# zhiyongggggg/dct-cryptonets

Measured on AMD Instinct MI355X. Metric: encrypted images/sec, ResNet-20 DCT-24x16^2 CIFAR-10, higher is better.
Workload: dtype u64 torus + f64 FFT (one-level tiers keep 32-bit accumulators)

## Files before the change

### dct-cryptonets_amd/csrc/dctfhe.hip

```cpp
#include <hip/hip_runtime.h>
#include <sys/random.h>

#include <algorithm>
#include <array>
#include <atomic>
#include <cmath>
#include <cstdarg>
#include <cstddef>
#include <cstdio>
#include <cstring>
#include <map>
#include <memory>
#include <string>
#include <vector>

#include "../../include/dctfhe.h"
#include "kernels.h"

using namespace dctfhe;

static thread_local std::string g_err;
static int fail(const char* fmt, ...) {
  char buf[1024];
  va_list ap;
// ... 350 lines not shown
  ~dctfhe_session() {
    if (ctx) hipSetDevice(ctx->device);
    wipe_audit_key();
  }
};

#define PBS_CASES(X)                                                                                 \
  X(8, 2, 2, 8) X(9, 1, 2, 16) X(9, 1, 3, 8) X(10, 1, 1, 8) X(10, 1, 2, 8) X(10, 2, 1, 8) X(10, 2, 2, 8)  \
  X(11, 1, 1, 8) X(11, 1, 2, 8) X(11, 1, 3, 8) X(12, 1, 1, 8) X(12, 1, 2, 8) X(12, 1, 3, 8)           \
  X(13, 1, 1, 8) X(13, 1, 2, 8) X(13, 1, 3, 8) X(11, 1, 4, 8)

#define PBS_MB_CASES(X) X(11) X(12) X(13)

template <int LOGN, int K_, int L_, int P>
constexpr int groups_for() {
  using G = pbs_geom<LOGN, K_, L_, P>;
  constexpr int by_lds = (160 * 1024 - G::TW_BYTES) / G::GROUP_BYTES;
  int g = G::T >= 256 ? 1 : 256 / G::T;
  while (g > 1 && g > by_lds) g >>= 1;
  while (g > 1 && 2 * (G::TW_BYTES + g * G::GROUP_BYTES) > 160 * 1024) g >>= 1;
  return g;
}

static int tier_ppt(const dctfhe_tier& t) {
#define X(LN, K_, L_, P_) if (t.logN == LN && t.k == K_ && t.l == L_) return P_;
  PBS_CASES(X)
#undef X
  return 0;
}

#define SET_LDS_ATTR(kernel, bytes)                                                                  \
  do {                                                                                               \
    static uint64_t done_mask = 0;                                                                   \
    int dev_ = 0;                                                                                    \
    HIPCHK(hipGetDevice(&dev_));                                                                     \
    if (dev_ < 0 || dev_ >= 64 || !((done_mask >> dev_) & 1)) {                                      \
      HIPCHK(hipFuncSetAttribute((const void*)(kernel), hipFuncAttributeMaxDynamicSharedMemorySize, (int)(bytes))); \
      if (dev_ >= 0 && dev_ < 64) done_mask |= 1ull << dev_;                                         \
    }                                                                                                \
  } while (0)

template <int LN, int K, int L, int P, int GR, int MB = 0>
static int launch_pbs_as(const pbs_launch& a, hipStream_t st) {
  const size_t lds = pbs_lds_bytes<LN, K, L, P, MB>(GR);
  SET_LDS_ATTR((pbs_kernel<LN, K, L, P, GR, MB>), lds);
  const unsigned grid = (unsigned)((a.count + GR - 1) / GR);
  hipLaunchKernelGGL((pbs_kernel<LN, K, L, P, GR, MB>), dim3(grid), dim3(pbs_geom<LN, K, L, P, MB>::T * GR), lds, st, a);
  HIPCHK(hipGetLastError());
  return 0;
}

static int launch_pbs(const dctfhe_tier& t, const pbs_launch& a, hipStream_t st) {
  if (a.count == 0) return 0;
  if (a.pf_parts != 0 && a.pf_parts < 8) return fail("bootstrap launch: pf_parts must be 0 or >= 8 (got %d)", a.pf_parts);
  if (!a.bsk || !a.tw || !a.cts_small || !a.out || !a.dummy || (t.unroll == 2 && !a.wtab)) return fail("bootstrap launch: null operand");
  if (a.w < 0 || a.w > t.logN - 1) return fail("bootstrap launch: table of 2^%d entries does not fit N = 2^%d", a.w, t.logN);
#define X(LN, K_, L_, P_) \
  if (t.logN == LN && t.k == K_ && t.l == L_ && t.unroll == 1) return launch_pbs_as<LN, K_, L_, P_, groups_for<LN, K_, L_, P_>()>(a, st);
  PBS_CASES(X)
#undef X
#define X(LN) \
  if (t.logN == LN && t.k == 1 && t.l == 1 && t.unroll == 2) return launch_pbs_as<LN, 1, 1, 8, (LN == 12 ? 2 : groups_for<LN, 1, 1, 8>()), 1>(a, st);
  PBS_MB_CASES(X)
#undef X
  if (t.logN == 11 && t.k == 1 && t.l == 3 && t.unroll == 2) return launch_pbs_as<11, 1, 3, 8, 4, 1>(a, st);
  if (t.logN == 10 && t.k == 2 && t.l == 1 && t.unroll == 2) return launch_pbs_as<10, 2, 1, 8, 4, 1>(a, st);
  return fail("no bootstrap kernel instantiated for logN=%d k=%d l=%d unroll=%d", t.logN, t.k, t.l, t.unroll);
}

static int make_twiddles(const dctfhe_tier& t, std::vector<cplx>& tw) {
#define X(LN, K_, L_, P_)                                        \
  if (t.logN == LN && t.k == K_ && t.l == L_) {                  \
    tw.resize(fft_geom<LN - 1, P_>::TW_ELEMS);                   \
    fill_twiddles<LN - 1, P_>(tw.data());                        \
    return 0;                                                    \
  }
  PBS_CASES(X)
#undef X
  return fail("no bootstrap kernel instantiated for logN=%d k=%d l=%d", t.logN, t.k, t.l);
}

static int launch_bsk_fourier(const dctfhe_tier& t, const uint64_t* polys, size_t npoly, const cplx* tw, cplx* out, hipStream_t st) {
#define X(LN, K_, L_, P_)                                                                            \
  if (t.logN == LN && t.k == K_ && t.l == L_) {                                                      \
    using F = fft_geom<LN - 1, P_>;                                                                  \
    constexpr int GR = groups_for<LN, K_, L_, P_>();                                                 \
    const size_t lds = (size_t)F::TW_ELEMS * 16 + (size_t)GR * F::EXCH_ELEMS * 16;                   \
    SET_LDS_ATTR((k_bsk_fourier<LN, P_, GR>), lds);                                                  \
    const unsigned grid = (unsigned)((npoly + GR - 1) / GR);                                         \
    hipLaunchKernelGGL((k_bsk_fourier<LN, P_, GR>), dim3(grid), dim3(F::T * GR), lds, st, polys, npoly, tw, out); \
    HIPCHK(hipGetLastError());                                                                       \
    return 0;                                                                                        \
  }
  PBS_CASES(X)
#undef X
  return fail("no bootstrap kernel instantiated for logN=%d k=%d l=%d", t.logN, t.k, t.l);
}

extern "C" int dctfhe_ctx_create(int device_id, dctfhe_ctx** out) {
  int ndev = 0;
  if (hipGetDeviceCount(&ndev) != hipSuccess || ndev <= 0)
    return fail("dctfhe: no HIP device visible -- this engine has no CPU path");
  if (device_id < 0 || device_id >= ndev) return fail("dctfhe: device %d out of range (%d visible)", device_id, ndev);
  HIPCHK(hipSetDevice(device_id));
  std::unique_ptr<dctfhe_ctx> c(new dctfhe_ctx);
// ... 275 lines not shown
    if (t.ksk_share < 0) n += tier_ksk_words(p, t) * 8;
    n += tier_bsk_elems(t) * sizeof(cplx);
  }
  return n;
}
extern "C" int dctfhe_eval_keys_export(dctfhe_eval_keys* E, void* buf, size_t capacity, size_t* size) {
  if (!E || !size) return fail("dctfhe_eval_keys_export: null argument");
  const size_t need = eval_blob_size(E->p);
  *size = need;
  if (!buf) return 0;
  if (capacity < need) return fail("dctfhe_eval_keys_export: buffer of %zu bytes, %zu needed", capacity, need);
  HIPCHK(hipSetDevice(E->ctx->device));
  HIPCHK(hipStreamSynchronize(E->ctx->stream));
  EvalBlobHeader h{};
  h.magic = 0x4b564544u ; h.version = EVAL_BLOB_VERSION; h.total_bytes = need; h.params = E->p;
  char* q = (char*)buf;
  memcpy(q, &h, sizeof h); q += sizeof h;
  for (int ti = 0; ti < E->p.n_tiers; ti++) {
    const dctfhe_tier& t = E->p.tiers[ti];
    if (t.ksk_share < 0) {
      HIPCHK(hipMemcpy(q, E->ksk[ti].ksk.p, tier_ksk_words(E->p, t) * 8, hipMemcpyDeviceToHost));
      q += tier_ksk_words(E->p, t) * 8;
    }
    HIPCHK(hipMemcpy(q, E->tiers[ti].bsk.p, tier_bsk_elems(t) * sizeof(cplx), hipMemcpyDeviceToHost));
    q += tier_bsk_elems(t) * sizeof(cplx);
  }
  return 0;
}
static constexpr uint32_t EVAL_CBLOB_MAGIC = 0x43564544u , EVAL_CBLOB_VERSION = 1;
static size_t eval_cblob_size(const dctfhe_params& p) {
  size_t n = sizeof(EvalBlobHeader) + 32;
  for (int ti = 0; ti < p.n_tiers; ti++) {
    const dctfhe_tier& t = p.tiers[ti];
    if (t.ksk_share < 0) n += (size_t)p.D * t.lk * 8;
    n += tier_bsk_body_words(t) * 8;
  }
  return n;
}
static void key_to_bytes(const rng_key& k, uint8_t* b) {
  for (int i = 0; i < 8; i++) for (int x = 0; x < 4; x++) b[4 * i + x] = (uint8_t)(k.k[i] >> (8 * x));
}
static uint64_t ksk_grid_mask(const dctfhe_tier& t) {
  const int drop = 64 - 8 * ks_limbs(t);
  return drop ? ~0ULL << drop : ~0ULL;
}
static int launch_expand(const rng_key& key, uint64_t stream, uint64_t row0, uint64_t stride, int dim_eff, uint64_t and_mask, const uint64_t* d_bodies,
                         int nb, size_t count, size_t L, uint64_t* d_out, hipStream_t st) {
// ... 132 lines not shown
  CHK(expand_bsk_chunk(pub, tier, t, 0, (int)tier_bsk_blocks(t), (const uint64_t*)q, d_b.as<uint64_t>(), d_std.as<uint64_t>(), ctx->stream));
  HIPCHK(d_std.download(out, body_bytes * (t.k + 1), ctx->stream));
  return 0;
}

extern "C" int dctfhe_eval_keys_import(dctfhe_ctx* ctx, const void* buf, size_t size, dctfhe_eval_keys** out) {
  if (!ctx || !buf || !out) return fail("dctfhe_eval_keys_import: null argument");
  if (size < sizeof(EvalBlobHeader)) return fail("evaluation-key blob too short");
  EvalBlobHeader h;
  memcpy(&h, buf, sizeof h);
  if (h.magic == EVAL_CBLOB_MAGIC) return import_compressed(ctx, buf, size, out);
  if (h.magic != 0x4b564544u || h.version != EVAL_BLOB_VERSION) return fail("bad evaluation-key blob magic/version");
  CHK(check_params(&h.params));
  if (h.total_bytes != size || eval_blob_size(h.params) != size) return fail("evaluation-key blob is %zu bytes, its parameters need %zu", size, eval_blob_size(h.params));
  std::unique_ptr<dctfhe_eval_keys> E;
  CHK(eval_alloc(ctx, &h.params, E));
  const char* q = (const char*)buf + sizeof h;
  for (int ti = 0; ti < h.params.n_tiers; ti++) {
    const dctfhe_tier& t = h.params.tiers[ti];
    if (t.ksk_share < 0) {
      HIPCHK(hipMemcpy(E->ksk[ti].ksk.p, q, tier_ksk_words(h.params, t) * 8, hipMemcpyHostToDevice));
      q += tier_ksk_words(h.params, t) * 8;
    }
    HIPCHK(hipMemcpy(E->tiers[ti].bsk.p, q, tier_bsk_elems(t) * sizeof(cplx), hipMemcpyHostToDevice));
    q += tier_bsk_elems(t) * sizeof(cplx);
  }
  CHK(eval_finish(E.get()));
  *out = E.release();
  return 0;
}

extern "C" int dctfhe_client_key_export_secret(dctfhe_client_key* C, uint8_t* big_key, uint8_t* small_key) {
  HIPCHK(hipSetDevice(C->ctx->device));
  HIPCHK(hipMemcpy(big_key, C->S(), C->p.D, hipMemcpyDeviceToHost));
  HIPCHK(hipMemcpy(small_key, C->s(), C->p.n_max, hipMemcpyDeviceToHost));
  return 0;
}
extern "C" int dctfhe_eval_keys_export_ksk(dctfhe_eval_keys* K, int tier, uint64_t* out) {
  if (tier < 0 || tier >= K->p.n_tiers) return fail("tier out of range");
  const dctfhe_tier& t = K->p.tiers[tier];
  HIPCHK(hipSetDevice(K->ctx->device));
  HIPCHK(hipMemcpy(out, K->tiers[tier].ks->ksk.p, (size_t)K->p.D * t.lk * (t.n + 1) * 8, hipMemcpyDeviceToHost));
  return 0;
}
extern "C" int dctfhe_client_key_export_bsk(dctfhe_client_key* C, int tier, uint64_t* out) {
  if (tier < 0 || tier >= C->p.n_tiers) return fail("tier out of range");
  const dctfhe_tier& t = C->p.tiers[tier];
// ... 2365 lines not shown
```

### dct-cryptonets_amd/csrc/fft_core.h

```cpp
#pragma once
#include <stdint.h>
#include <type_traits>

#if defined(__HIPCC__)
#define HD __host__ __device__ __forceinline__
#else
#define HD inline __attribute__((always_inline))
#endif

namespace dctfhe {

struct cplx { double re, im; };

struct no_tick { template <int K> HD void at() {} };
#if defined(__HIP_DEVICE_COMPILE__) && defined(DCTFHE_PHASE_TIMERS)
struct phase_clock {
  unsigned long long last, acc[12];
  __device__ __forceinline__ void start() { for (int k = 0; k < 12; k++) acc[k] = 0; last = __builtin_amdgcn_s_memtime(); }
  template <int K> __device__ __forceinline__ void at() { const unsigned long long now = __builtin_amdgcn_s_memtime(); acc[K] += now - last; last = now; }
};
#endif

HD cplx cmk(double re, double im) { cplx c; c.re = re; c.im = im; return c; }
HD cplx cadd(cplx a, cplx b) { return cmk(a.re + b.re, a.im + b.im); }
// ... 66 lines not shown
      y[0] = cadd(a, b); y[1] = csub(a, b);
    } else {
      cplx e[R / 2], o[R / 2];
      small_dft<R / 2, 2 * S, SIGN>::run(x, e);
      small_dft<R / 2, 2 * S, SIGN>::run(x + S, o);
      static_for<0, R / 2>([&](auto K) {
        constexpr int k = decltype(K)::value;
        const cplx t = mul_root64<k*(64 / R), SIGN>(o[k]);
        y[k] = cadd(e[k], t); y[k + R / 2] = csub(e[k], t);
      });
    }
  }
};

HD void fused_bf(const cplx a, const cplx b, const double tr, const double ti, cplx& p, cplx& m) {
  p.re = __builtin_fma(tr, b.re, __builtin_fma(-ti, b.im, a.re));
  p.im = __builtin_fma(tr, b.im, __builtin_fma(ti, b.re, a.im));
  m.re = __builtin_fma(2.0, a.re, -p.re);
  m.im = __builtin_fma(2.0, a.im, -p.im);
}
template <int R, int S, int LV>
struct fused_idft {
  static HD void run(const cplx* x, cplx* y, const cplx* pw, const cplx cw8) {
    static_assert(R == 2 || R == 4 || R == 8, "radix 8 passes");
    if constexpr (R == 2) {
      fused_bf(x[0], x[S], pw[LV].re, pw[LV].im, y[0], y[1]);
    } else {
      cplx e[R / 2], o[R / 2];
      fused_idft<R / 2, 2 * S, LV + 1>::run(x, e, pw, cw8);
      fused_idft<R / 2, 2 * S, LV + 1>::run(x + S, o, pw, cw8);
      const cplx c = pw[LV];
      fused_bf(e[0], o[0], c.re, c.im, y[0], y[R / 2]);
      if constexpr (R == 4) {
        fused_bf(e[1], o[1], -c.im, c.re, y[1], y[1 + R / 2]);
      } else {
        fused_bf(e[1], o[1], cw8.re, cw8.im, y[1], y[1 + R / 2]);
        fused_bf(e[2], o[2], -c.im, c.re, y[2], y[2 + R / 2]);
        fused_bf(e[3], o[3], -cw8.im, cw8.re, y[3], y[3 + R / 2]);
      }
    }
  }
};
HD void fused_idft_factors(const cplx b, cplx* pw, cplx& cw8) {
  constexpr double h = 0.70710678118654752440;
  pw[0] = cmk(b.re, -b.im);
  pw[1] = csqr(pw[0]);
  pw[2] = csqr(pw[1]);
// ... 11 lines not shown
  return w;
}
constexpr int geom_tw_offset(int LOGM, int P, int i) {
  int o = 0;
  for (int j = 0; j < i; j++) o += geom_weight(LOGM, P, j);
  return o;
}

template <int LOGM, int P>
struct fft_geom {
  static constexpr int M = 1 << LOGM;
  static_assert(geom_logp(P) > 0, "P must be 4, 8 or 16");
  static constexpr int T = M / P;
  static constexpr int S = geom_passes(LOGM, P);
  static_assert(S >= 2, "need at least two passes");
  static constexpr int radix(int i) { return geom_radix(LOGM, P, i); }
  static constexpr int weight(int i) { return geom_weight(LOGM, P, i); }
  static constexpr int tw_offset(int i) { return geom_tw_offset(LOGM, P, i); }
  static constexpr int TW_TOTAL = geom_tw_offset(LOGM, P, S - 1);
  static constexpr int TW_ELEMS = TW_TOTAL + T;
  static HD int skew(int idx) { return idx + (idx >> geom_logp(P)); }
  static HD int swz(int idx) { return (idx >> 9) * 576 + ((idx & 511) ^ ((idx >> 3) & 7)); }
  static constexpr bool swz_reader(int i) { return P == 8 && LOGM >= 10 && geom_radix(LOGM, P, i) == P && geom_weight(LOGM, P, i) >= 16; }
  template <int IR> static HD int ex(int idx) { if constexpr (swz_reader(IR)) return swz(idx); else return skew(idx); }
  static constexpr int EXCH_ELEMS = M + (M >> geom_logp(P));
};

HD int pass_base(int W, int R, int t) { return (t / W) * (W * R) + (t % W); }

template <int LOGM, int P, int I>
HD int pass_addr(int t, int j) {
  using G = fft_geom<LOGM, P>;
  constexpr int R = G::radix(I), W = G::weight(I);
  if constexpr (R == P) return pass_base(W, R, t) + j * W;
  else return P * t + j;
}

struct no_hook { HD void operator()() const {} };

template <int LOGM, int P, class Sync, class WSync, class Hook = no_hook>
HD void fft_forward(cplx* v, int t, const cplx* tw, const cplx twist, cplx* exch, Sync&& sync, WSync&& wsync, Hook&& before_last = Hook{}) {
  using G = fft_geom<LOGM, P>;
  constexpr int S = G::S;
  static_for<0, P>([&](auto J) { constexpr int j = decltype(J)::value; v[j] = mul_root64<j*(64 / (4 * P)), +1>(v[j]); });
  static_for<0, S>([&](auto I) {
    constexpr int i = decltype(I)::value;
    constexpr int R = G::radix(i);
    constexpr int W = G::weight(i);
    if constexpr (i == S - 1) before_last();
    cplx y[P];
    if constexpr (R == P) {
      small_dft<P, 1, -1>::run(v, y);
    } else {
      static_for<0, P / R>([&](auto Gp) { constexpr int g = decltype(Gp)::value; small_dft<R, 1, -1>::run(v + g * R, y + g * R); });
    }
    if constexpr (i < S - 1) {
      const cplx b = tw[G::tw_offset(i) + (t % W)];
      {
        cplx run = (i == 0) ? twist : cmk(1.0, 0.0);
        if constexpr (i == 0) y[0] = cmul(y[0], run);
        static_for<1, R>([&](auto K) { constexpr int k = decltype(K)::value; run = cmul(run, b); y[k] = cmul(y[k], run); });
      }
      if constexpr (W <= 64) wsync(); else sync();
      static_for<0, P>([&](auto J) { constexpr int j = decltype(J)::value; exch[G::template ex<i + 1>(pass_addr<LOGM, P, i>(t, j))] = y[j]; });
      if constexpr (W <= 64) wsync(); else sync();
      static_for<0, P>([&](auto J) { constexpr int j = decltype(J)::value; v[j] = exch[G::template ex<i + 1>(pass_addr<LOGM, P, i + 1>(t, j))]; });
    } else {
      static_for<0, P>([&](auto J) { constexpr int j = decltype(J)::value; v[j] = y[j]; });
    }
  });
}

template <int LOGM, int P, class Sync, class WSync>
HD void fft_inverse(cplx* v, int t, const cplx* tw, const cplx twist, cplx* exch, Sync&& sync, WSync&& wsync) {
  using G = fft_geom<LOGM, P>;
  constexpr int S = G::S;
  static_for<0, S>([&](auto Irev) {
    constexpr int i = S - 1 - decltype(Irev)::value;
    constexpr int R = G::radix(i);
    constexpr int W = G::weight(i);
    constexpr bool FUSED = i > 0 && i < S - 1 && R == P && P == 8;
    if constexpr (i < S - 1 && !FUSED) {
      const cplx b = tw[G::tw_offset(i) + (t % W)];
      {
        cplx run = (i == 0) ? twist : cmk(1.0, 0.0);
        if constexpr (i == 0) v[0] = cmulc(v[0], run);
        static_for<1, R>([&](auto K) { constexpr int k = decltype(K)::value; run = cmul(run, b); v[k] = cmulc(v[k], run); });
      }
    }
    cplx y[P];
    if constexpr (FUSED) {
      cplx pw[3], cw8;
      fused_idft_factors(tw[G::tw_offset(i) + (t % W)], pw, cw8);
      fused_idft<P, 1, 0>::run(v, y, pw, cw8);
    } else if constexpr (R == P) {
      small_dft<P, 1, +1>::run(v, y);
    } else {
      static_for<0, P / R>([&](auto Gp) { constexpr int g = decltype(Gp)::value; small_dft<R, 1, +1>::run(v + g * R, y + g * R); });
    }
    if constexpr (i > 0) {
      constexpr int Wp = G::weight(i - 1);
      static_for<0, P>([&](auto J) { constexpr int j = decltype(J)::value; exch[G::template ex<i - 1>(pass_addr<LOGM, P, i>(t, j))] = y[j]; });
      if constexpr (Wp <= 64) wsync(); else sync();
      static_for<0, P>([&](auto J) { constexpr int j = decltype(J)::value; v[j] = exch[G::template ex<i - 1>(pass_addr<LOGM, P, i - 1>(t, j))]; });
      if constexpr (Wp <= 64) wsync(); else sync();
    } else {
      static_for<0, P>([&](auto J) { constexpr int j = decltype(J)::value; v[j] = mul_root64<j*(64 / (4 * P)), -1>(y[j]); });
    }
  });
}

template <int LOGM, int P, int NP, class Sync, class WSync, class Tick = no_tick>
HD void fft_forward_n(cplx (&v)[NP][P], int t, const cplx* tw, const cplx twist, cplx* exch, Sync&& sync, WSync&& wsync, Tick&& tick = Tick{}) {
  using G = fft_geom<LOGM, P>;
  constexpr int S = G::S;
  static_for<0, NP>([&](auto U) {
    constexpr int u = decltype(U)::value;
    static_for<0, P>([&](auto J) { constexpr int j = decltype(J)::value; v[u][j] = mul_root64<j*(64 / (4 * P)), +1>(v[u][j]); });
  });
  static_for<0, S>([&](auto I) {
    constexpr int i = decltype(I)::value;
    constexpr int R = G::radix(i);
    constexpr int W = G::weight(i);
    if constexpr (i < S - 1) {
      const cplx b = tw[G::tw_offset(i) + (t % W)];
      const cplx run0 = (i == 0) ? twist : cmk(1.0, 0.0);
      if constexpr (W > 64) tick.template at<0>();
      if constexpr (W <= 64) wsync(); else sync();
      if constexpr (W > 64) tick.template at<1>();
      cplx y[NP][P];
      static_for<0, NP>([&](auto U) { constexpr int u = decltype(U)::value; small_dft<P, 1, -1>::run(v[u], y[u]); });
      {
        cplx run = run0;
        if constexpr (i == 0) static_for<0, NP>([&](auto U) { constexpr int u = decltype(U)::value; y[u][0] = cmul(y[u][0], run); });
        static_for<1, R>([&](auto K) {
          constexpr int k = decltype(K)::value;
          run = cmul(run, b);
          static_for<0, NP>([&](auto U) { constexpr int u = decltype(U)::value; y[u][k] = cmul(y[u][k], run); });
        });
      }
      static_for<0, NP>([&](auto U) {
        constexpr int u = decltype(U)::value;
        cplx* ex = exch + u * G::EXCH_ELEMS;
        static_for<0, P>([&](auto J) { constexpr int j = decltype(J)::value; ex[G::template ex<i + 1>(pass_addr<LOGM, P, i>(t, j))] = y[u][j]; });
      });
      if constexpr (W > 64) tick.template at<2>();
      if constexpr (W <= 64) wsync(); else sync();
      if constexpr (W > 64) tick.template at<3>();
      static_for<0, NP>([&](auto U) {
        constexpr int u = decltype(U)::value;
        const cplx* ex = exch + u * G::EXCH_ELEMS;
        static_for<0, P>([&](auto J) { constexpr int j = decltype(J)::value; v[u][j] = ex[G::template ex<i + 1>(pass_addr<LOGM, P, i + 1>(t, j))]; });
      });
    } else {
      static_for<0, NP>([&](auto U) {
        constexpr int u = decltype(U)::value;
        cplx y[P];
        if constexpr (R == P) {
          small_dft<P, 1, -1>::run(v[u], y);
        } else {
          static_for<0, P / R>([&](auto Gp) { constexpr int g = decltype(Gp)::value; small_dft<R, 1, -1>::run(v[u] + g * R, y + g * R); });
        }
        static_for<0, P>([&](auto J) { constexpr int j = decltype(J)::value; v[u][j] = y[j]; });
      });
    }
  });
  tick.template at<4>();
}

template <int LOGM, int P, int NP, class Sync, class WSync, class Tick = no_tick>
HD void fft_inverse_n(cplx (&v)[NP][P], int t, const cplx* tw, const cplx twist, cplx* exch, Sync&& sync, WSync&& wsync, Tick&& tick = Tick{}) {
  using G = fft_geom<LOGM, P>;
  constexpr int S = G::S;
  static_for<0, S>([&](auto Irev) {
    constexpr int i = S - 1 - decltype(Irev)::value;
    constexpr int R = G::radix(i);
    constexpr int W = G::weight(i);
    if constexpr (i > 0 && G::weight(i > 0 ? i - 1 : 0) > 64) tick.template at<6>();
    cplx b = cmk(1.0, 0.0), run0 = cmk(1.0, 0.0);
    if constexpr (i < S - 1) {
      b = tw[G::tw_offset(i) + (t % W)];
      if constexpr (i == 0) run0 = twist;
    }
    constexpr bool FUSED = i > 0 && i < S - 1 && R == P && P == 8;
    [[maybe_unused]] cplx pw[3], cw8;
    if constexpr (FUSED) fused_idft_factors(b, pw, cw8);
    if constexpr (i < S - 1 && !FUSED) {
      cplx run = run0;
      if constexpr (i == 0) static_for<0, NP>([&](auto U) { constexpr int u = decltype(U)::value; v[u][0] = cmulc(v[u][0], run); });
      static_for<1, R>([&](auto K) {
        constexpr int k = decltype(K)::value;
        run = cmul(run, b);
        static_for<0, NP>([&](auto U) { constexpr int u = decltype(U)::value; v[u][k] = cmulc(v[u][k], run); });
      });
    }
    static_for<0, NP>([&](auto U) {
      constexpr int u = decltype(U)::value;
      cplx y[P];
      if constexpr (FUSED) {
        fused_idft<P, 1, 0>::run(v[u], y, pw, cw8);
      } else if constexpr (R == P) {
        small_dft<P, 1, +1>::run(v[u], y);
      } else {
        static_for<0, P / R>([&](auto Gp) { constexpr int g = decltype(Gp)::value; small_dft<R, 1, +1>::run(v[u] + g * R, y + g * R); });
      }
      if constexpr (i > 0) {
        cplx* ex = exch + u * G::EXCH_ELEMS;
        static_for<0, P>([&](auto J) { constexpr int j = decltype(J)::value; ex[G::template ex<i - 1>(pass_addr<LOGM, P, i>(t, j))] = y[j]; });
      } else {
        static_for<0, P>([&](auto J) { constexpr int j = decltype(J)::value; v[u][j] = mul_root64<j*(64 / (4 * P)), -1>(y[j]); });
      }
    });
    if constexpr (i > 0) {
      constexpr int Wp = G::weight(i - 1);
      if constexpr (Wp > 64) tick.template at<7>();
      if constexpr (Wp <= 64) wsync(); else sync();
      if constexpr (Wp > 64) tick.template at<8>();
      static_for<0, NP>([&](auto U) {
        constexpr int u = decltype(U)::value;
        const cplx* ex = exch + u * G::EXCH_ELEMS;
        static_for<0, P>([&](auto J) { constexpr int j = decltype(J)::value; v[u][j] = ex[G::template ex<i - 1>(pass_addr<LOGM, P, i - 1>(t, j))]; });
      });
      if constexpr (Wp > 64) tick.template at<9>();
      if constexpr (Wp <= 64) wsync(); else sync();
      if constexpr (Wp > 64) tick.template at<10>();
    }
  });
}

template <int LOGM, int P>
HD int spectrum_freq(int p) {
  int k = 0, fw = 1;
  for (int i = 0; i < geom_passes(LOGM, P); i++) {
    const int W = geom_weight(LOGM, P, i), R = geom_radix(LOGM, P, i);
    k += ((p / W) % R) * fw;
    fw *= R;
  }
  return k;
}

template <int LOGM, int P>
inline void fill_twiddles(cplx* tw) {
  using G = fft_geom<LOGM, P>;
  const long double PI = 3.141592653589793238462643383279502884L;
// ... 38 lines not shown
```

### dct-cryptonets_amd/csrc/kernels.h

```cpp
#pragma once
#include <hip/hip_runtime.h>
#include "pbs_core.h"
#include "client_shared.h"

namespace dctfhe {

__device__ __forceinline__ int64_t gauss_torus(const rng_key& key, uint64_t stream, uint64_t idx, double sigma) {
  if (sigma <= 0.0) return 0;
  return gauss_torus_words(rnd64(key, stream, 2 * idx), rnd64(key, stream, 2 * idx + 1), sigma);
}

__global__ void k_gen_bits(rng_key key, uint64_t stream, uint8_t* out, int len) {
  const int i = blockIdx.x * blockDim.x + threadIdx.x;
  if (i < len) out[i] = (uint8_t)(rnd64(key, stream, (uint64_t)i) >> 63);
}
__global__ void k_rng_fill(rng_key key, uint64_t stream, uint64_t idx0, uint64_t* out, size_t count) {
  const size_t i = (size_t)blockIdx.x * blockDim.x + threadIdx.x;
  if (i < count) out[i] = rnd64(key, stream, idx0 + i);
}

__device__ __forceinline__ uint64_t block_reduce_add(uint64_t v, uint64_t* red) {
  for (int off = 32; off > 0; off >>= 1) v += __shfl_down(v, off);
  const int lane = threadIdx.x & 63, wv = threadIdx.x >> 6;
  if (lane == 0) red[wv] = v;
// ... 687 lines not shown
  pbs_args A;
  A.ct_small = a.cts_small + e * (size_t)(a.n + 1);
  A.n = a.n; A.beta = a.beta; A.bsk = a.bsk;
  const size_t ti = a.table_idx ? (size_t)a.table_idx[e] : (a.nchan > 1 ? ((a.e_offset + e) / (size_t)a.hw) % (size_t)a.nchan : 0);
  A.table = a.tables + (ti << a.w);
  A.w = a.w;
  A.out = live ? a.out + e * (size_t)(a.D_out + 1) : a.dummy;
  A.D_out = a.D_out;
  A.accumulate = live ? a.accumulate : 0;
  A.body_add = a.body_add;
  A.bsk_wrap = a.bsk_wrap;
  A.pf_parts = a.pf_parts;
  A.wtab = a.wtab;
  A.zlut = MB ? tw + G::TW_LDS_ELEMS : nullptr;
  if constexpr (G::TWIST_LDS) A.twist = tw + G::F::TW_TOTAL; else A.twist = a.tw + G::F::TW_TOTAL;
  A.pf_rank = (int)((blockIdx.x / 8) % (unsigned)(a.pf_parts > 0 ? a.pf_parts : 1));
  if constexpr (T <= 64) {
    pbs_thread<LOGN, K, L, P, MB>(A, t, tw, stage, exch, accl, pf_dump, [] { __builtin_amdgcn_wave_barrier(); }, [] { __builtin_amdgcn_wave_barrier(); });
  } else {
    pbs_thread<LOGN, K, L, P, MB>(A, t, tw, stage, exch, accl, pf_dump, [] { __syncthreads(); }, [] { __builtin_amdgcn_wave_barrier(); });
  }
}

template <int COT>
__global__ void __launch_bounds__(256)
k_conv2d(const uint64_t* __restrict__ in, int Cin, int H, int W, size_t Lin, size_t Deff, const int8_t* __restrict__ wgt, int c0, int c1,
         int pix0, int KH, int KW, int stride, int pad, int Ho, int Wo, size_t Lout, uint64_t* __restrict__ out) {
  const size_t word = (size_t)blockIdx.x * 256 + threadIdx.x;
  const int pix = pix0 + blockIdx.y;
  const int co0 = c0 + blockIdx.z * COT;
  const int b = pix / (Ho * Wo), y = (pix / Wo) % Ho, x = pix % Wo;
  if (word >= Lout) return;
  const bool body = word == Lout - 1;
  uint64_t acc[COT];
#pragma unroll
  for (int c = 0; c < COT; c++) acc[c] = 0;
  if (body || word < Deff) {
    const size_t iw = body ? Lin - 1 : word;
    const uint64_t* inb = in + (size_t)b * Cin * H * W * Lin;
    for (int ci = 0; ci < Cin; ci++)
      for (int ky = 0; ky < KH; ky++) {
        const int iy = y * stride + ky - pad;
        if (iy < 0 || iy >= H) continue;
        for (int kx = 0; kx < KW; kx++) {
          const int ix = x * stride + kx - pad;
          if (ix < 0 || ix >= W) continue;
// ... 335 lines not shown
```

### dct-cryptonets_amd/csrc/pbs_core.h

```cpp
#pragma once
#include "fft_core.h"

namespace dctfhe {

#if defined(__HIP_DEVICE_COMPILE__)
#define DCTFHE_SCHED_BARRIER() __builtin_amdgcn_sched_barrier(0)
#define DCTFHE_UNIFORM(x) ((uint32_t)__builtin_amdgcn_readfirstlane((int)(x)))
#define DCTFHE_DEVICE 1
#else
#define DCTFHE_SCHED_BARRIER() ((void)0)
#define DCTFHE_UNIFORM(x) (x)
#endif

constexpr int PBS_KEY_BATCH = 4;
constexpr int PBS_PF_DIST = 2;

template <int LOGN, int K, int L, int P, int MB = 0>
struct pbs_geom {
  static constexpr int N = 1 << LOGN;
  static constexpr int LOGM = LOGN - 1;
  static constexpr int M = N / 2;
  using F = fft_geom<LOGM, P>;
  static constexpr int T = F::T;
  static constexpr int ROWS = (K + 1) * L;
// ... 439 lines not shown
  if (blockIdx.x == DCTFHE_PHASE_TIMERS && (threadIdx.x & 63) == 0)
    for (int k = 0; k < 12; k++) dctfhe_phase_ticks[(threadIdx.x >> 6) * 12 + k] = tick.acc[k];
#endif
  uint64_t* o = A.out;
  static_for<0, K>([&](auto Pp) {
    constexpr int p = decltype(Pp)::value;
    static_for<0, 2 * P>([&](auto R) {
      constexpr int r = decltype(R)::value;
      const int c = t + T * r;
      const int dst = p * N + (c == 0 ? 0 : N - c);
      uint64_t av;
      if constexpr (p < NL) av = acc_wide(accl[p * N + c]); else av = acc_wide(acc[p][r]);
      const uint64_t v = (c == 0) ? av : (uint64_t)0 - av;
      if (A.accumulate) o[dst] += v; else o[dst] = v;
    });
  });
  if (!A.accumulate)
    for (int j = K * N + t; j < A.D_out; j += T) o[j] = 0;
  if (t == 0) {
    if (A.accumulate) o[A.D_out] += acc_wide(acc[K][0]) + A.body_add; else o[A.D_out] = acc_wide(acc[K][0]) + A.body_add;
  }
}

template <int LOGN, int P, class Sync, class WSync>
HD void key_poly_to_fourier(const uint64_t* poly, cplx* dst, int t, const cplx* tw, cplx* exch, Sync&& sync, WSync&& wsync) {
  constexpr int N = 1 << LOGN, M = N / 2;
  using F = fft_geom<LOGN - 1, P>;
  constexpr int T = F::T;
  cplx v[P];
  static_for<0, P>([&](auto J) {
    constexpr int j = decltype(J)::value;
    v[j] = cmk((double)(int64_t)poly[t + T * j], (double)(int64_t)poly[t + T * j + M]);
  });
  fft_forward<LOGN - 1, P>(v, t, tw, tw[F::TW_TOTAL + t], exch, sync, wsync);
  const double inv = 0x1p-64 / (double)M;
  static_for<0, P>([&](auto J) { constexpr int j = decltype(J)::value; dst[j * T + t] = cmk(v[j].re * inv, v[j].im * inv); });
}

}
```

Baseline: 0.08425.

## Add duo PBS kernel sharing each key load across two ciphertexts for logN=11 l=3 tier

Adds a new bootstrap kernel for the logN=11, k=1, l=3 two-bit tier in which each thread group processes two ciphertexts at once. Each key-bundle load is reused for both ciphertexts, and the FFT runs at 4 points per thread (twice the threads per polynomial) with batched n=2 transforms. The fused radix-4 idft path and a new XOR swizzle for the P=4 exchange buffer support this. The bootstrap key in device memory now has a different spectral ordering, so export and import permute it on the host. The aim is to halve key bandwidth per ciphertext, at the cost of more registers and LDS per group and lower occupancy.

```diff
diff --git a/dct-cryptonets_amd/csrc/dctfhe.hip b/dct-cryptonets_amd/csrc/dctfhe.hip
--- a/dct-cryptonets_amd/csrc/dctfhe.hip
+++ b/dct-cryptonets_amd/csrc/dctfhe.hip
@@ -396,6 +396,28 @@
   return g;
 }
 
+static bool tier_duo(const dctfhe_tier& t) { return t.logN == 11 && t.k == 1 && t.l == 3 && t.unroll == 2; }
+constexpr int DUO_LOGN = 11, DUO_P = 4, DUO_BLOB_P = 8, DUO_M = 1 << (DUO_LOGN - 1);
+static const std::vector<uint16_t>& duo_entry_map() {
+  static const std::vector<uint16_t> map = [] {
+    std::vector<uint16_t> by_freq(DUO_M), m(DUO_M);
+    constexpr int T4 = DUO_M / DUO_P, T8 = DUO_M / DUO_BLOB_P;
+    for (int e = 0; e < DUO_M; e++) by_freq[spectrum_freq<DUO_LOGN - 1, DUO_P>(DUO_P * (e % T4) + e / T4)] = (uint16_t)e;
+    for (int e = 0; e < DUO_M; e++) m[e] = by_freq[spectrum_freq<DUO_LOGN - 1, DUO_BLOB_P>(DUO_BLOB_P * (e % T8) + e / T8)];
+    return m;
+  }();
+  return map;
+}
+static void duo_permute(const cplx* src, cplx* dst, size_t npoly, bool to_device) {
+  const std::vector<uint16_t>& m = duo_entry_map();
+  for (size_t q = 0; q < npoly; q++) {
+    const cplx* a = src + q * DUO_M;
+    cplx* b = dst + q * DUO_M;
+    if (to_device) for (int e = 0; e < DUO_M; e++) b[m[e]] = a[e];
+    else           for (int e = 0; e < DUO_M; e++) b[e] = a[m[e]];
+  }
+}
+
 static int tier_ppt(const dctfhe_tier& t) {
 #define X(LN, K_, L_, P_) if (t.logN == LN && t.k == K_ && t.l == L_) return P_;
   PBS_CASES(X)
@@ -420,6 +442,17 @@
   SET_LDS_ATTR((pbs_kernel<LN, K, L, P, GR, MB>), lds);
   const unsigned grid = (unsigned)((a.count + GR - 1) / GR);
   hipLaunchKernelGGL((pbs_kernel<LN, K, L, P, GR, MB>), dim3(grid), dim3(pbs_geom<LN, K, L, P, MB>::T * GR), lds, st, a);
+  HIPCHK(hipGetLastError());
+  return 0;
+}
+
+template <int LN, int K, int L, int P, int DUOS>
+static int launch_pbs_as_duo(const pbs_launch& a, hipStream_t st) {
+  const size_t lds = pbs_duo_lds_bytes<LN, K, L, P>(DUOS);
+  static_assert(pbs_duo_lds_bytes<LN, K, L, P>(DUOS) <= 160 * 1024, "LDS of one CU");
+  SET_LDS_ATTR((pbs_kernel_duo<LN, K, L, P, DUOS>), lds);
+  const unsigned grid = (unsigned)((a.count + 2 * DUOS - 1) / (2 * DUOS));
+  hipLaunchKernelGGL((pbs_kernel_duo<LN, K, L, P, DUOS>), dim3(grid), dim3(pbs_geom<LN, K, L, P, 1>::T * DUOS), lds, st, a);
   HIPCHK(hipGetLastError());
   return 0;
 }
@@ -437,12 +470,18 @@
   if (t.logN == LN && t.k == 1 && t.l == 1 && t.unroll == 2) return launch_pbs_as<LN, 1, 1, 8, (LN == 12 ? 2 : groups_for<LN, 1, 1, 8>()), 1>(a, st);
   PBS_MB_CASES(X)
 #undef X
-  if (t.logN == 11 && t.k == 1 && t.l == 3 && t.unroll == 2) return launch_pbs_as<11, 1, 3, 8, 4, 1>(a, st);
+  static_assert(DUO_LOGN == 11 && DUO_P == 4, "tier_duo names this kernel's shape");
+  if (t.logN == 11 && t.k == 1 && t.l == 3 && t.unroll == 2) return launch_pbs_as_duo<11, 1, 3, 4, 2>(a, st);
   if (t.logN == 10 && t.k == 2 && t.l == 1 && t.unroll == 2) return launch_pbs_as<10, 2, 1, 8, 4, 1>(a, st);
   return fail("no bootstrap kernel instantiated for logN=%d k=%d l=%d unroll=%d", t.logN, t.k, t.l, t.unroll);
 }
 
 static int make_twiddles(const dctfhe_tier& t, std::vector<cplx>& tw) {
+  if (tier_duo(t)) {
+    tw.resize(fft_geom<DUO_LOGN - 1, DUO_P>::TW_ELEMS);
+    fill_twiddles<DUO_LOGN - 1, DUO_P>(tw.data());
+    return 0;
+  }
 #define X(LN, K_, L_, P_)                                        \
   if (t.logN == LN && t.k == K_ && t.l == L_) {                  \
     tw.resize(fft_geom<LN - 1, P_>::TW_ELEMS);                   \
@@ -455,6 +494,14 @@
 }
 
 static int launch_bsk_fourier(const dctfhe_tier& t, const uint64_t* polys, size_t npoly, const cplx* tw, cplx* out, hipStream_t st) {
+  if (tier_duo(t)) {
+    using F = fft_geom<DUO_LOGN - 1, DUO_P>;
+    const size_t lds = (size_t)F::TW_ELEMS * 16 + (size_t)F::EXCH_ELEMS * 16;
+    SET_LDS_ATTR((k_bsk_fourier<DUO_LOGN, DUO_P, 1>), lds);
+    hipLaunchKernelGGL((k_bsk_fourier<DUO_LOGN, DUO_P, 1>), dim3((unsigned)npoly), dim3(F::T), lds, st, polys, npoly, tw, out);
+    HIPCHK(hipGetLastError());
+    return 0;
+  }
 #define X(LN, K_, L_, P_)                                                                            \
   if (t.logN == LN && t.k == K_ && t.l == L_) {                                                      \
     using F = fft_geom<LN - 1, P_>;                                                                  \
@@ -776,7 +823,13 @@
       HIPCHK(hipMemcpy(q, E->ksk[ti].ksk.p, tier_ksk_words(E->p, t) * 8, hipMemcpyDeviceToHost));
       q += tier_ksk_words(E->p, t) * 8;
     }
-    HIPCHK(hipMemcpy(q, E->tiers[ti].bsk.p, tier_bsk_elems(t) * sizeof(cplx), hipMemcpyDeviceToHost));
+    if (tier_duo(t)) {
+      std::vector<cplx> dev(tier_bsk_elems(t));
+      HIPCHK(hipMemcpy(dev.data(), E->tiers[ti].bsk.p, dev.size() * sizeof(cplx), hipMemcpyDeviceToHost));
+      duo_permute(dev.data(), (cplx*)q, dev.size() / DUO_M, false);
+    } else {
+      HIPCHK(hipMemcpy(q, E->tiers[ti].bsk.p, tier_bsk_elems(t) * sizeof(cplx), hipMemcpyDeviceToHost));
+    }
     q += tier_bsk_elems(t) * sizeof(cplx);
   }
   return 0;
@@ -955,7 +1008,13 @@
       HIPCHK(hipMemcpy(E->ksk[ti].ksk.p, q, tier_ksk_words(h.params, t) * 8, hipMemcpyHostToDevice));
       q += tier_ksk_words(h.params, t) * 8;
     }
-    HIPCHK(hipMemcpy(E->tiers[ti].bsk.p, q, tier_bsk_elems(t) * sizeof(cplx), hipMemcpyHostToDevice));
+    if (tier_duo(t)) {
+      std::vector<cplx> dev(tier_bsk_elems(t));
+      duo_permute((const cplx*)q, dev.data(), dev.size() / DUO_M, true);
+      HIPCHK(hipMemcpy(E->tiers[ti].bsk.p, dev.data(), dev.size() * sizeof(cplx), hipMemcpyHostToDevice));
+    } else {
+      HIPCHK(hipMemcpy(E->tiers[ti].bsk.p, q, tier_bsk_elems(t) * sizeof(cplx), hipMemcpyHostToDevice));
+    }
     q += tier_bsk_elems(t) * sizeof(cplx);
   }
   CHK(eval_finish(E.get()));
diff --git a/dct-cryptonets_amd/csrc/fft_core.h b/dct-cryptonets_amd/csrc/fft_core.h
--- a/dct-cryptonets_amd/csrc/fft_core.h
+++ b/dct-cryptonets_amd/csrc/fft_core.h
@@ -112,7 +112,7 @@
 template <int R, int S, int LV>
 struct fused_idft {
   static HD void run(const cplx* x, cplx* y, const cplx* pw, const cplx cw8) {
-    static_assert(R == 2 || R == 4 || R == 8, "radix 8 passes");
+    static_assert(R == 2 || R == 4 || R == 8, "radix 4 and radix 8 passes");
     if constexpr (R == 2) {
       fused_bf(x[0], x[S], pw[LV].re, pw[LV].im, y[0], y[1]);
     } else {
@@ -170,7 +170,12 @@
   static HD int skew(int idx) { return idx + (idx >> geom_logp(P)); }
   static HD int swz(int idx) { return (idx >> 9) * 576 + ((idx & 511) ^ ((idx >> 3) & 7)); }
   static constexpr bool swz_reader(int i) { return P == 8 && LOGM >= 10 && geom_radix(LOGM, P, i) == P && geom_weight(LOGM, P, i) >= 16; }
-  template <int IR> static HD int ex(int idx) { if constexpr (swz_reader(IR)) return swz(idx); else return skew(idx); }
+  static HD int x4(int idx) { return idx ^ ((idx >> 2) & 3) ^ (((idx >> 4) & 3) << 2); }
+  template <int IR, int E> static HD int ex(int idx) {
+    if constexpr (P == 4) { if constexpr (E < 2) return idx; else return x4(idx); }
+    else if constexpr (swz_reader(IR)) return swz(idx);
+    else return skew(idx);
+  }
   static constexpr int EXCH_ELEMS = M + (M >> geom_logp(P));
 };
 
@@ -210,9 +215,9 @@
         static_for<1, R>([&](auto K) { constexpr int k = decltype(K)::value; run = cmul(run, b); y[k] = cmul(y[k], run); });
       }
       if constexpr (W <= 64) wsync(); else sync();
-      static_for<0, P>([&](auto J) { constexpr int j = decltype(J)::value; exch[G::template ex<i + 1>(pass_addr<LOGM, P, i>(t, j))] = y[j]; });
+      static_for<0, P>([&](auto J) { constexpr int j = decltype(J)::value; exch[G::template ex<i + 1, i>(pass_addr<LOGM, P, i>(t, j))] = y[j]; });
       if constexpr (W <= 64) wsync(); else sync();
-      static_for<0, P>([&](auto J) { constexpr int j = decltype(J)::value; v[j] = exch[G::template ex<i + 1>(pass_addr<LOGM, P, i + 1>(t, j))]; });
+      static_for<0, P>([&](auto J) { constexpr int j = decltype(J)::value; v[j] = exch[G::template ex<i + 1, i>(pass_addr<LOGM, P, i + 1>(t, j))]; });
     } else {
       static_for<0, P>([&](auto J) { constexpr int j = decltype(J)::value; v[j] = y[j]; });
     }
@@ -227,7 +232,7 @@
     constexpr int i = S - 1 - decltype(Irev)::value;
     constexpr int R = G::radix(i);
     constexpr int W = G::weight(i);
-    constexpr bool FUSED = i > 0 && i < S - 1 && R == P && P == 8;
+    constexpr bool FUSED = i > 0 && i < S - 1 && R == P && (P == 8 || P == 4);
     if constexpr (i < S - 1 && !FUSED) {
       const cplx b = tw[G::tw_offset(i) + (t % W)];
       {
@@ -248,9 +253,9 @@
     }
     if constexpr (i > 0) {
       constexpr int Wp = G::weight(i - 1);
-      static_for<0, P>([&](auto J) { constexpr int j = decltype(J)::value; exch[G::template ex<i - 1>(pass_addr<LOGM, P, i>(t, j))] = y[j]; });
+      static_for<0, P>([&](auto J) { constexpr int j = decltype(J)::value; exch[G::template ex<i - 1, i - 1>(pass_addr<LOGM, P, i>(t, j))] = y[j]; });
       if constexpr (Wp <= 64) wsync(); else sync();
-      static_for<0, P>([&](auto J) { constexpr int j = decltype(J)::value; v[j] = exch[G::template ex<i - 1>(pass_addr<LOGM, P, i - 1>(t, j))]; });
+      static_for<0, P>([&](auto J) { constexpr int j = decltype(J)::value; v[j] = exch[G::template ex<i - 1, i - 1>(pass_addr<LOGM, P, i - 1>(t, j))]; });
       if constexpr (Wp <= 64) wsync(); else sync();
     } else {
       static_for<0, P>([&](auto J) { constexpr int j = decltype(J)::value; v[j] = mul_root64<j*(64 / (4 * P)), -1>(y[j]); });
@@ -290,7 +295,7 @@
       static_for<0, NP>([&](auto U) {
         constexpr int u = decltype(U)::value;
         cplx* ex = exch + u * G::EXCH_ELEMS;
-        static_for<0, P>([&](auto J) { constexpr int j = decltype(J)::value; ex[G::template ex<i + 1>(pass_addr<LOGM, P, i>(t, j))] = y[u][j]; });
+        static_for<0, P>([&](auto J) { constexpr int j = decltype(J)::value; ex[G::template ex<i + 1, i>(pass_addr<LOGM, P, i>(t, j))] = y[u][j]; });
       });
       if constexpr (W > 64) tick.template at<2>();
       if constexpr (W <= 64) wsync(); else sync();
@@ -298,7 +303,7 @@
       static_for<0, NP>([&](auto U) {
         constexpr int u = decltype(U)::value;
         const cplx* ex = exch + u * G::EXCH_ELEMS;
-        static_for<0, P>([&](auto J) { constexpr int j = decltype(J)::value; v[u][j] = ex[G::template ex<i + 1>(pass_addr<LOGM, P, i + 1>(t, j))]; });
+        static_for<0, P>([&](auto J) { constexpr int j = decltype(J)::value; v[u][j] = ex[G::template ex<i + 1, i>(pass_addr<LOGM, P, i + 1>(t, j))]; });
       });
     } else {
       static_for<0, NP>([&](auto U) {
@@ -330,7 +335,7 @@
       b = tw[G::tw_offset(i) + (t % W)];
       if constexpr (i == 0) run0 = twist;
     }
-    constexpr bool FUSED = i > 0 && i < S - 1 && R == P && P == 8;
+    constexpr bool FUSED = i > 0 && i < S - 1 && R == P && (P == 8 || P == 4);
     [[maybe_unused]] cplx pw[3], cw8;
     if constexpr (FUSED) fused_idft_factors(b, pw, cw8);
     if constexpr (i < S - 1 && !FUSED) {
@@ -354,7 +359,7 @@
       }
       if constexpr (i > 0) {
         cplx* ex = exch + u * G::EXCH_ELEMS;
-        static_for<0, P>([&](auto J) { constexpr int j = decltype(J)::value; ex[G::template ex<i - 1>(pass_addr<LOGM, P, i>(t, j))] = y[j]; });
+        static_for<0, P>([&](auto J) { constexpr int j = decltype(J)::value; ex[G::template ex<i - 1, i - 1>(pass_addr<LOGM, P, i>(t, j))] = y[j]; });
       } else {
         static_for<0, P>([&](auto J) { constexpr int j = decltype(J)::value; v[u][j] = mul_root64<j*(64 / (4 * P)), -1>(y[j]); });
       }
@@ -367,7 +372,7 @@
       static_for<0, NP>([&](auto U) {
         constexpr int u = decltype(U)::value;
         const cplx* ex = exch + u * G::EXCH_ELEMS;
-        static_for<0, P>([&](auto J) { constexpr int j = decltype(J)::value; v[u][j] = ex[G::template ex<i - 1>(pass_addr<LOGM, P, i - 1>(t, j))]; });
+        static_for<0, P>([&](auto J) { constexpr int j = decltype(J)::value; v[u][j] = ex[G::template ex<i - 1, i - 1>(pass_addr<LOGM, P, i - 1>(t, j))]; });
       });
       if constexpr (Wp > 64) tick.template at<9>();
       if constexpr (Wp <= 64) wsync(); else sync();
diff --git a/dct-cryptonets_amd/csrc/kernels.h b/dct-cryptonets_amd/csrc/kernels.h
--- a/dct-cryptonets_amd/csrc/kernels.h
+++ b/dct-cryptonets_amd/csrc/kernels.h
@@ -733,6 +733,58 @@
   }
 }
 
+template <int LOGN, int K, int L, int P>
+constexpr size_t pbs_duo_lds_bytes(int duos) {
+  using G = pbs_geom<LOGN, K, L, P, 1>;
+  return (size_t)G::TW_BYTES + (size_t)duos * 2 * G::GROUP_BYTES;
+}
+
+template <int LOGN, int K, int L, int P, int DUOS>
+__global__ void __launch_bounds__((pbs_geom<LOGN, K, L, P, 1>::T * DUOS), ((pbs_geom<LOGN, K, L, P, 1>::T * DUOS) >= 512 ? 1 : 2))
+pbs_kernel_duo(pbs_launch a) {
+  using G = pbs_geom<LOGN, K, L, P, 1>;
+  constexpr int T = G::T;
+  static_assert(T >= 64 && T % 64 == 0, "a wave holds threads of one duo only");
+  static_assert(G::TWIST_LDS && G::SHARED_BYTES == G::EXCH_BYTES, "duo LDS layout");
+  extern __shared__ __attribute__((aligned(16))) unsigned char smem_raw[];
+  cplx* tw = reinterpret_cast<cplx*>(smem_raw);
+  unsigned char* per_duo = smem_raw + G::TW_BYTES;
+  for (int x = threadIdx.x; x < G::TW_LDS_ELEMS; x += blockDim.x) tw[x] = a.tw[x];
+  {
+    cplx* zl = tw + G::TW_LDS_ELEMS;
+    for (int x = threadIdx.x; x < G::ZLUT_ELEMS; x += blockDim.x) zl[x] = x < (1 << G::ZLO) ? a.wtab[x] : a.wtab[(size_t)(x - (1 << G::ZLO)) << G::ZLO];
+  }
+  __syncthreads();
+  const int g = threadIdx.x / T, t = threadIdx.x % T;
+  unsigned char* mine = per_duo + (size_t)g * 2 * G::GROUP_BYTES;
+  cplx* exch = reinterpret_cast<cplx*>(mine);
+  uint64_t* accl = reinterpret_cast<uint64_t*>(mine + 2 * G::EXCH_BYTES);
+  pbs_args A2[2];
+#pragma unroll
+  for (int c = 0; c < 2; c++) {
+    size_t e = ((size_t)blockIdx.x * DUOS + g) * 2 + c;
+    const bool live = e < a.count;
+    if (!live) e = a.count - 1;
+    pbs_args& A = A2[c];
+    A.ct_small = a.cts_small + e * (size_t)(a.n + 1);
+    A.n = a.n; A.beta = a.beta; A.bsk = a.bsk;
+    const size_t ti = a.table_idx ? (size_t)a.table_idx[e] : (a.nchan > 1 ? ((a.e_offset + e) / (size_t)a.hw) % (size_t)a.nchan : 0);
+    A.table = a.tables + (ti << a.w);
+    A.w = a.w;
+    A.out = live ? a.out + e * (size_t)(a.D_out + 1) : a.dummy;
+    A.D_out = a.D_out;
+    A.accumulate = live ? a.accumulate : 0;
+    A.body_add = a.body_add;
+    A.bsk_wrap = 0;
+    A.pf_parts = a.pf_parts;
+    A.wtab = a.wtab;
+    A.zlut = tw + G::TW_LDS_ELEMS;
+    A.twist = tw + G::F::TW_TOTAL;
+    A.pf_rank = (int)((blockIdx.x / 8) % (unsigned)(a.pf_parts > 0 ? a.pf_parts : 1));
+  }
+  pbs_thread_duo<LOGN, K, L, P>(A2, t, tw, exch, accl, nullptr, [] { __syncthreads(); }, [] { __builtin_amdgcn_wave_barrier(); });
+}
+
 template <int COT>
 __global__ void __launch_bounds__(256)
 k_conv2d(const uint64_t* __restrict__ in, int Cin, int H, int W, size_t Lin, size_t Deff, const int8_t* __restrict__ wgt, int c0, int c1,
diff --git a/dct-cryptonets_amd/csrc/pbs_core.h b/dct-cryptonets_amd/csrc/pbs_core.h
--- a/dct-cryptonets_amd/csrc/pbs_core.h
+++ b/dct-cryptonets_amd/csrc/pbs_core.h
@@ -485,6 +485,203 @@
   }
 }
 
+template <int LOGN, int K, int L, int P, class Sync, class WSync>
+HD void pbs_thread_duo(const pbs_args (&A2)[2], int t, const cplx* tw, cplx* exch, uint64_t* accl_raw, uint32_t* pf_dump, Sync&& sync, WSync&& wsync) {
+  using G = pbs_geom<LOGN, K, L, P, 1>;
+  static_assert(!G::PAIR && !G::ACC32, "the duo is the general two-bit form");
+  static_assert(G::NG == 1, "one small transform per thread in the last pass: a single monomial base per exponent");
+  constexpr int N = G::N, M = G::M, T = G::T, NL = G::NL;
+  using acc_t = typename G::acc_t;
+  const pbs_args& A = A2[0];
+  acc_t* const accl = reinterpret_cast<acc_t*>(accl_raw);
+  const int n = A.n;
+  const int msh = 64 - LOGN - 2;
+  const cplx twist = A.twist[t];
+
+  constexpr int PF_LINES = (int)(G::KEY_BLOCKS * G::BSK_ELEMS_PER_KEYBIT * 16 / 128);
+  constexpr int PF_ROUNDS = (PF_LINES / 8 + T - 1) / T;
+  const char* pf_ptr;
+  const size_t pf_step = (size_t)G::KEY_BLOCKS * G::BSK_ELEMS_PER_KEYBIT * 16;
+  {
+    const int parts = A.pf_parts >= 8 ? A.pf_parts : PF_LINES;
+    const int per = (PF_LINES + parts - 1) / parts;
+    int line = A.pf_rank * per + (t < per ? t : per - 1);
+    if (line > PF_LINES - 1 - (PF_ROUNDS - 1) * T) line = PF_LINES - 1 - (PF_ROUNDS - 1) * T;
+    if (line < 0) line = 0;
+    pf_ptr = reinterpret_cast<const char*>(A.bsk) + (size_t)PBS_PF_DIST * pf_step + (size_t)line * 128;
+  }
+  acc_t acc[2][K + 1][2 * P];
+  static_for<0, 2>([&](auto Cc) {
+    constexpr int c = decltype(Cc)::value;
+    const uint32_t bt = (uint32_t)(((A2[c].ct_small[n] >> msh) + 1) >> 1) & (2 * N - 1);
+    static_for<0, K>([&](auto Pp) {
+      constexpr int p = decltype(Pp)::value;
+      static_for<0, 2 * P>([&](auto R) {
+        constexpr int r = decltype(R)::value;
+        if constexpr (p < NL) accl[(c * NL + p) * N + t + T * r] = 0; else acc[c][p][r] = 0;
+      });
+    });
+    static_for<0, 2 * P>([&](auto R) {
+      constexpr int r = decltype(R)::value;
+      const uint32_t idx = ((uint32_t)(t + T * r) + bt) & (2 * N - 1);
+      const uint64_t v = testvec_coeff(A2[c].table, A2[c].w, N, (int)(idx & (N - 1)));
+      acc[c][K][r] = (acc_t)((idx & N) ? (uint64_t)0 - v : v);
+    });
+  });
+
+  const uint32_t ulow0 = (uint32_t)(1 - 4 * spectrum_freq<G::LOGM, P>(P * t)) & (2 * N - 1);
+  auto zeta = [&](uint32_t m) -> cplx {
+#if defined(DCTFHE_DEVICE)
+    return cmul(A.zlut[(1 << G::ZLO) + (m >> G::ZLO)], A.zlut[m & ((1u << G::ZLO) - 1)]);
+#else
+    return A.zlut ? cmul(A.zlut[(1 << G::ZLO) + (m >> G::ZLO)], A.zlut[m & ((1u << G::ZLO) - 1)]) : A.wtab[m];
+#endif
+  };
+#if defined(__HIP_DEVICE_COMPILE__) && defined(DCTFHE_PHASE_TIMERS)
+  phase_clock tick;
+  tick.start();
+#else
+  no_tick tick;
+#endif
+  for (int i = 0; i < n; i += 2) {
+    uint32_t au[2], a2u[2], e1[2], e2[2];
+    static_for<0, 2>([&](auto Cc) {
+      constexpr int c = decltype(Cc)::value;
+      const uint32_t a = (uint32_t)(((A2[c].ct_small[i] >> msh) + 1) >> 1) & (2 * N - 1);
+      const uint32_t a2 = (uint32_t)(((A2[c].ct_small[i + 1] >> msh) + 1) >> 1) & (2 * N - 1);
+      au[c] = DCTFHE_UNIFORM(a); a2u[c] = DCTFHE_UNIFORM(a2);
+      e1[c] = a * ulow0; e2[c] = a2 * ulow0;
+    });
+    const cplx* key = A.bsk + (size_t)(3 * (i >> 1)) * G::BSK_ELEMS_PER_KEYBIT;
+    cplx out[K + 1][2][P];
+    static_for<0, K + 1>([&](auto Pp) {
+      constexpr int p = decltype(Pp)::value;
+      uint32_t packed[2][2 * P];
+      double first[2][2 * P];
+      static_for<0, 2>([&](auto Cc) {
+        constexpr int c = decltype(Cc)::value;
+        static_for<0, 2 * P>([&](auto R) {
+          constexpr int r = decltype(R)::value;
+          acc_t own;
+          if constexpr (p < NL) own = accl[(c * NL + p) * N + t + T * r]; else own = acc[c][p][r];
+          int32_t dg[L];
+          decompose<L>(own, A.beta, dg);
+          first[c][r] = (double)dg[0];
+          packed[c][r] = pack_digits<L>(dg);
+        });
+      });
+      static_for<0, L>([&](auto Lv) {
+        constexpr int lev = decltype(Lv)::value;
+        constexpr int row = p * L + lev;
+        cplx v[2][P];
+        static_for<0, 2>([&](auto Cc) {
+          constexpr int c = decltype(Cc)::value;
+          static_for<0, P>([&](auto J) {
+            constexpr int j = decltype(J)::value;
+            if constexpr (lev == 0) v[c][j] = cmk(first[c][j], first[c][P + j]);
+            else v[c][j] = cmk(unpack_digit<L, lev>(packed[c][j]), unpack_digit<L, lev>(packed[c][P + j]));
+          });
+        });
+        fft_forward_n<G::LOGM, P, 2>(v, t, tw, twist, exch, sync, wsync, tick);
+        cplx zb1[2], zb2[2];
+        static_for<0, 2>([&](auto Cc) {
+          constexpr int c = decltype(Cc)::value;
+          zb1[c] = zeta(e1[c] & (2 * N - 1));
+          zb2[c] = zeta(e2[c] & (2 * N - 1));
+        });
+        static_for<0, P>([&](auto J) {
+          constexpr int j = decltype(J)::value;
+          cplx kk[3][K + 1];
+          static_for<0, 3>([&](auto Ww) {
+            constexpr int w = decltype(Ww)::value;
+            static_for<0, K + 1>([&](auto Q) {
+              constexpr int q = decltype(Q)::value;
+              kk[w][q] = load_uniform_base(key + (((size_t)w * G::ROWS * (K + 1) + (size_t)row * (K + 1) + q) * M + j * T), (unsigned)t);
+            });
+          });
+          DCTFHE_SCHED_BARRIER();
+          static_for<0, 2>([&](auto Cc) {
+            constexpr int c = decltype(Cc)::value;
+            cplx z1 = zb1[c], z2 = zb2[c];
+            if constexpr (j > 0) {
+              z1 = cmul(z1, root8((0u - au[c] * (uint32_t)j) * (8 / P)));
+              z2 = cmul(z2, root8((0u - a2u[c] * (uint32_t)j) * (8 / P)));
+            }
+            const cplx m1 = cmk(z1.re - 1.0, z1.im), m2 = cmk(z2.re - 1.0, z2.im);
+            cplx m12 = cmul(z1, z2); m12.re -= 1.0;
+            static_for<0, K + 1>([&](auto Q) {
+              constexpr int q = decltype(Q)::value;
+              const cplx bundle = cfma(m12, kk[2][q], cfma(m2, kk[1][q], cmul(m1, kk[0][q])));
+              if constexpr (row == 0) out[q][c][j] = cmul(v[c][j], bundle); else out[q][c][j] = cfma(v[c][j], bundle, out[q][c][j]);
+            });
+          });
+          DCTFHE_SCHED_BARRIER();
+        });
+        tick.template at<5>();
+      });
+    });
+
+    {
+      uint32_t acc_pf = 0;
+      static_for<0, PF_ROUNDS>([&](auto Rr) { acc_pf ^= *reinterpret_cast<const uint32_t*>(pf_ptr + (size_t)decltype(Rr)::value * T * 128); });
+#if defined(__HIP_DEVICE_COMPILE__)
+      asm volatile("" ::"v"(acc_pf));
+#else
+      pf_dump[t] = acc_pf;
+#endif
+      pf_ptr += pf_step;
+    }
+    tick.template at<5>();
+
+    static_for<0, K + 1>([&](auto Q) {
+      constexpr int q = decltype(Q)::value;
+      fft_inverse_n<G::LOGM, P, 2>(out[q], t, tw, twist, exch, sync, wsync, tick);
+      static_for<0, 2>([&](auto Cc) {
+        constexpr int c = decltype(Cc)::value;
+        static_for<0, P>([&](auto J) {
+          constexpr int j = decltype(J)::value;
+          if constexpr (q < NL) {
+            acc_add(accl[(c * NL + q) * N + t + T * j], out[q][c][j].re);
+            acc_add(accl[(c * NL + q) * N + t + T * (P + j)], out[q][c][j].im);
+          } else {
+            acc_add(acc[c][q][j], out[q][c][j].re);
+            acc_add(acc[c][q][P + j], out[q][c][j].im);
+          }
+        });
+      });
+    });
+    tick.template at<11>();
+  }
+
+#if defined(__HIP_DEVICE_COMPILE__) && defined(DCTFHE_PHASE_TIMERS)
+  tick.template at<0>();
+  if (blockIdx.x == DCTFHE_PHASE_TIMERS && (threadIdx.x & 63) == 0)
+    for (int k = 0; k < 12; k++) dctfhe_phase_ticks[(threadIdx.x >> 6) * 12 + k] = tick.acc[k];
+#endif
+  static_for<0, 2>([&](auto Cc) {
+    constexpr int c = decltype(Cc)::value;
+    const pbs_args& B = A2[c];
+    uint64_t* o = B.out;
+    static_for<0, K>([&](auto Pp) {
+      constexpr int p = decltype(Pp)::value;
+      static_for<0, 2 * P>([&](auto R) {
+        constexpr int r = decltype(R)::value;
+        const int cf = t + T * r;
+        const int dst = p * N + (cf == 0 ? 0 : N - cf);
+        uint64_t av;
+        if constexpr (p < NL) av = acc_wide(accl[(c * NL + p) * N + cf]); else av = acc_wide(acc[c][p][r]);
+        const uint64_t v = (cf == 0) ? av : (uint64_t)0 - av;
+        if (B.accumulate) o[dst] += v; else o[dst] = v;
+      });
+    });
+    if (!B.accumulate)
+      for (int j = K * N + t; j < B.D_out; j += T) o[j] = 0;
+    if (t == 0) {
+      if (B.accumulate) o[B.D_out] += acc_wide(acc[c][K][0]) + B.body_add; else o[B.D_out] = acc_wide(acc[c][K][0]) + B.body_add;
+    }
+  });
+}
+
 template <int LOGN, int P, class Sync, class WSync>
 HD void key_poly_to_fourier(const uint64_t* poly, cplx* dst, int t, const cplx* tw, cplx* exch, Sync&& sync, WSync&& wsync) {
   constexpr int N = 1 << LOGN, M = N / 2;
```

New measurement: 0.08571, median of 6. 1.02x the previous value.
